# carlanton/cilium

Measured on AMD Instinct MI355X. Metric: Mpps classified (whole node) + % HBM roofline, 1/2/4/8 MI355X, higher is better.
Workload: dtype u32

## Files before the change

cilium_amd/csrc/gf_kernels.hip:

```cpp
#include "gf_internal.h"
#include "gf_device.h"
#include <rocprim/device/device_radix_sort.hpp>
#include <rocprim/device/device_scan.hpp>
#include <rocprim/device/device_run_length_encode.hpp>
#include <rocprim/device/device_select.hpp>
#include <rocprim/iterator/discard_iterator.hpp>
#include <rocprim/iterator/counting_iterator.hpp>
#include <errno.h>
#include <stdlib.h>
#include <stdio.h>
#include <functional>
#include <unordered_set>
#include <chrono>
#include <algorithm>
#include <array>
#include <atomic>
#include <string.h>

using namespace gf;
using namespace gfd;

#define BLOCK 256
#ifndef GF_DIAG
#define GF_DIAG 0
// ... 1668 lines not shown
    }
    if (stats && !(GF_DIAG & 2)) {
#if GF_ING_BINS_WAVE
        st.bins_wave(true, o.reason, o.action);
#else
        st.add(o.reason); st.add(256 + o.action);
#endif
        ln.sc.add(r.len, ab, o.ct_ret & 3u, st);
    }
}

__device__ __forceinline__ gf_rec ld_rec(const gf_rec *rec, uint32_t i) {
    if constexpr (GF_REC_NT) {
        const uint4 a = gload_nt16(rec + i), b = gload_nt16(reinterpret_cast<const uint8_t *>(rec + i) + 16);
        gf_rec r;
        __builtin_memcpy(&r, &a, 16);
        __builtin_memcpy(reinterpret_cast<uint8_t *>(&r) + 16, &b, 16);
        return r;
    } else {
        return rec[i];
    }
}
__device__ __forceinline__ void flush_added(const IngCtx &X, uint32_t fam_bit, int added, uint32_t *ct_count,
                                            uint32_t *lds_added) {
    if (X.strict & fam_bit) return;
    if (added) atomicAdd(lds_added, (uint32_t)added);
    __syncthreads();
    if (threadIdx.x == 0 && *lds_added && ct_count) atomicAdd(ct_count, *lds_added);
}

#ifndef GF_NCLS
#define GF_NCLS 1u
#endif
#define GF_NL (2u * GF_NCLS)
#define GF_LCAP 1024u
#define GF_SCHED_HIST(p) (p)
#define GF_SCHED_BASE(p) ((p) + GF_NL * (GF_LCAP + 1))
#define GF_SCHED_CURSOR(p) ((p) + 2 * GF_NL * (GF_LCAP + 1))
#define GF_SCHED_NRUNS(p) ((p) + 3 * GF_NL * (GF_LCAP + 1))
#define GF_SCHED_QUEUE(p) (GF_SCHED_NRUNS(p) + 1)
#define GF_SCHED_NFAM(p) (GF_SCHED_QUEUE(p) + GF_NL)
#define GF_SCHED_LCNT(p) (GF_SCHED_NFAM(p) + 2)
#define GF_SCHED_LSTART(p) (GF_SCHED_LCNT(p) + GF_NL)
#define GF_SCHED_WORDS (3 * GF_NL * (GF_LCAP + 1) + 1 + GF_NL + 2 + 2 * GF_NL)
#define GF_SCHED_HBYTES (GF_NL * (GF_LCAP + 1) * 4)
__device__ __forceinline__ uint32_t sched_list(uint32_t key, const gf_rec *rec, const uint32_t *perm, uint32_t b) {
    const uint32_t f = key >> (GF_KEY_BITS - 1);
    const uint32_t x = rec ? (uint32_t)rec[perm[b]].ep % GF_NCLS : 0u;
    return f * GF_NCLS + x;
}

template <int FAM, int GRAB = 1, bool PCT = false, bool RL = false>
__global__ __launch_bounds__(BLOCK, FAM == 6 ? GF_ING_MINW6 : GF_ING_MINW) void k_ing_groups(IngCtx X, uint32_t *sched, const uint2 *order,
                                                      const uint32_t *perm,
                                                      const gf_rec *rec, gf_ingress_out *out, uint32_t *ct_count,
                                                      unsigned long long *stats) {
    constexpr int F = FAM == 6 ? 1 : 0;
    const uint32_t *nfam = GF_SCHED_NFAM(sched);
    if (nfam[F] == 0) return;
    __shared__ uint32_t sl[272];
    __shared__ uint32_t sadd;
    Stats st{sl};
    if (threadIdx.x == 0) sadd = 0;
    if (stats) st.init(); else __syncthreads();
    const uint32_t lane = threadIdx.x & 63u;
    const uint32_t *lcnt = GF_SCHED_LCNT(sched), *lstart = GF_SCHED_LSTART(sched);
    __shared__ Lane<FAM> lanes[BLOCK];
    Lane<FAM> &ln = lanes[threadIdx.x];
    ln.init();
    uint32_t *const rlog = RL && X.rlog && !(X.rlog_off && *X.rlog_off) ? X.rlog : nullptr;
    const uint32_t x0 = blockIdx.x % GF_NCLS;
    for (uint32_t xi = 0; xi < GF_NCLS; xi++) {
    const uint32_t L = F * GF_NCLS + (x0 + xi) % GF_NCLS;
    uint32_t *queue = GF_SCHED_QUEUE(sched) + L;
    const uint32_t nb = lcnt[L];
    const uint2 *lorder = order + lstart[L];
    uint32_t grab = 1, gbase = 0, left = 0;
    for (;;) {
        uint32_t t;
        bool first = false;
        if constexpr (GRAB == 1) {
            uint32_t base = 0;
            if (lane == 0) base = atomicAdd(queue, 64u);
            base = __shfl(base, 0);
            if (base >= nb) break;
            t = base + lane;
        } else {
            if (!left) {
                uint32_t b0 = 0;
                if (lane == 0) b0 = atomicAdd(queue, 64u * grab);
                gbase = (uint32_t)__builtin_amdgcn_readfirstlane((int)b0);
                left = grab;
            }
            if (gbase >= nb) break;
            t = gbase + lane;
            first = left == grab;
            gbase += 64u; left--;
        }
        if (t >= nb) continue;
        const uint2 oc = lorder[t];
        if (GRAB > 1 && first && (uint32_t)__builtin_amdgcn_readfirstlane((int)oc.y) == 1u) grab = GRAB;
        const uint32_t b = oc.x, c = oc.y;
        uint32_t i = perm[b];
        uint32_t inx = c > 1 ? perm[b + 1] : 0u;
        gf_rec r = ld_rec(rec, i);
        lane_rel_drop<FAM, PCT>(X, ln);
// ... 135 lines not shown
        act = !(r.cls & 8) && (all || (r.ep && (gload<uint32_t>(&X.cfgs[r.ep - 1].flags) & GF_LXC_F_NO_CONNTRACK)));
        if (act) {
            len = r.len; ab = 8;
            o = handle_policy_noct(X, r, i, ab);
            if (X.pout && X.pout_wo) {
                uint8_t *q = X.pout + 24 * (size_t)i;
                const uint32_t ff = ((uint32_t)(r.cls >> 4) & 7u) << 5;
                *reinterpret_cast<uint32_t *>(q) = GF_STAGE_POLICY | ((uint32_t)o.action << 8) | ((uint32_t)o.reason << 16) |
                                                   ((uint32_t)o.ct_ret << 24);
                *reinterpret_cast<uint32_t *>(q + 4) = (ff | o.flags) | ((uint32_t)o.proxy_port << 16);
                *reinterpret_cast<uint16_t *>(q + 8) = o.ifindex_lo;
            } else if (X.pout) {
                uint8_t *q = X.pout + 24 * (size_t)i;
                uint2 a = *reinterpret_cast<const uint2 *>(q);
                uint2 b = *reinterpret_cast<const uint2 *>(q + 8);
                a.x = (a.x & 0xffu) | ((uint32_t)o.action << 8) | ((uint32_t)o.reason << 16) | ((uint32_t)o.ct_ret << 24);
                a.y = ((a.y & 0xffu) | o.flags) | (a.y & 0xff00u) | ((uint32_t)o.proxy_port << 16);
                b.x = (b.x & 0xffff0000u) | o.ifindex_lo;
                *reinterpret_cast<uint2 *>(q) = a;
                *reinterpret_cast<uint2 *>(q + 8) = b;
            } else {
                out[i] = o;
            }
        }
    }
    if (stats) {
        st.pkt_wave(act, o.reason, o.action, len, ab);
        const uint32_t c = (uint32_t)__popcll(__ballot(act));
        if ((threadIdx.x & 63u) == 0) st.add_n(264, c);
        st.flush(stats);
    }
}

#define GF_LCAP 1024u
#define GF_SCHED_ITEMS 4096
__global__ __launch_bounds__(BLOCK) void k_bucket_hist(uint32_t n, const uint32_t *off, const uint32_t *skeys,
                                                       const gf_rec *rec, const uint32_t *perm, uint32_t *sched) {
    extern __shared__ uint32_t h[];
    for (uint32_t k = threadIdx.x; k < GF_NL * (GF_LCAP + 1); k += blockDim.x) h[k] = 0;
    __syncthreads();
    uint32_t nq = *GF_SCHED_NRUNS(sched);
    uint32_t b0 = blockIdx.x * GF_SCHED_ITEMS;
    for (uint32_t q = b0 + threadIdx.x; q < b0 + GF_SCHED_ITEMS && q < nq; q += blockDim.x) {
        const uint32_t key = skeys[off[q]];
        uint32_t c = (q + 1 < nq ? off[q + 1] : n) - off[q];
        if (c && key != GF_KEY_SKIP)
            atomicAdd(&h[sched_list(key, rec, perm, off[q]) * (GF_LCAP + 1) + (c < GF_LCAP ? c : GF_LCAP)], 1u);
    }
    __syncthreads();
    uint32_t *hist = GF_SCHED_HIST(sched);
    for (uint32_t k = threadIdx.x; k < GF_NL * (GF_LCAP + 1); k += blockDim.x)
        if (h[k]) atomicAdd(&hist[k], h[k]);
}

__global__ __launch_bounds__(GF_LCAP) void k_bucket_base(uint32_t *sched) {
    __shared__ uint32_t s[GF_LCAP];
    __shared__ uint32_t tot;
    const uint32_t k = threadIdx.x, c = GF_LCAP - k;
    const uint32_t *hist = GF_SCHED_HIST(sched);
    uint32_t *base = GF_SCHED_BASE(sched), *cursor = GF_SCHED_CURSOR(sched);
    if (k == 0) { tot = 0; GF_SCHED_NFAM(sched)[0] = GF_SCHED_NFAM(sched)[1] = 0; }
    __syncthreads();
    for (uint32_t l = 0; l < GF_NL; l++) {
        const uint32_t *hf = hist + l * (GF_LCAP + 1);
        s[k] = hf[c];
        __syncthreads();
        for (uint32_t d = 1; d < GF_LCAP; d <<= 1) {
            uint32_t v = k >= d ? s[k - d] : 0u;
            __syncthreads();
            s[k] += v;
            __syncthreads();
        }
        const uint32_t add = tot;
        base[l * (GF_LCAP + 1) + c] = add + s[k] - hf[c];
        cursor[l * (GF_LCAP + 1) + c] = 0;
        if (k == 0) { base[l * (GF_LCAP + 1)] = add; cursor[l * (GF_LCAP + 1)] = 0; }
        __syncthreads();
        if (k == GF_LCAP - 1) {
            GF_SCHED_LCNT(sched)[l] = s[k];
            GF_SCHED_LSTART(sched)[l] = add;
            GF_SCHED_NFAM(sched)[l / GF_NCLS] += s[k];
            GF_SCHED_QUEUE(sched)[l] = 0;
            tot = add + s[k];
        }
        __syncthreads();
    }
}

__global__ __launch_bounds__(BLOCK) void k_bucket_order(uint32_t n, const uint32_t *off, const uint32_t *skeys,
                                                        const gf_rec *rec, const uint32_t *perm, uint32_t *sched,
                                                        uint2 *order, uint32_t skip1) {
    extern __shared__ uint32_t h[];
    for (uint32_t k = threadIdx.x; k < GF_NL * (GF_LCAP + 1); k += blockDim.x) h[k] = 0;
    __syncthreads();
    uint32_t nq = *GF_SCHED_NRUNS(sched);
    const uint32_t *base = GF_SCHED_BASE(sched);
    uint32_t *cursor = GF_SCHED_CURSOR(sched);
    uint32_t b0 = blockIdx.x * GF_SCHED_ITEMS;
    for (uint32_t q = b0 + threadIdx.x; q < b0 + GF_SCHED_ITEMS && q < nq; q += blockDim.x) {
        const uint32_t key = skeys[off[q]];
        uint32_t c = (q + 1 < nq ? off[q + 1] : n) - off[q];
        if (c && key != GF_KEY_SKIP && !(skip1 && c == 1))
            atomicAdd(&h[sched_list(key, rec, perm, off[q]) * (GF_LCAP + 1) + (c < GF_LCAP ? c : GF_LCAP)], 1u);
    }
    __syncthreads();
    for (uint32_t k = threadIdx.x; k < GF_NL * (GF_LCAP + 1); k += blockDim.x)
        if (h[k]) h[k] = base[k] + atomicAdd(&cursor[k], h[k]);
    __syncthreads();
    for (uint32_t q = b0 + threadIdx.x; q < b0 + GF_SCHED_ITEMS && q < nq; q += blockDim.x) {
        const uint32_t key = skeys[off[q]];
        uint32_t c = (q + 1 < nq ? off[q + 1] : n) - off[q];
        if (c && key != GF_KEY_SKIP && !(skip1 && c == 1))
            order[atomicAdd(&h[sched_list(key, rec, perm, off[q]) * (GF_LCAP + 1) + (c < GF_LCAP ? c : GF_LCAP)], 1u)] =
                make_uint2(off[q], c);
    }
}
__global__ __launch_bounds__(BLOCK) void k_single_mark(uint32_t n, const uint32_t *off, const uint32_t *skeys,
                                                       const uint32_t *perm, const uint32_t *sched, uint32_t *sw) {
    const uint32_t nq = *GF_SCHED_NRUNS(sched);
    for (uint32_t q = blockIdx.x * BLOCK + threadIdx.x; q < nq; q += gridDim.x * BLOCK) {
        const uint32_t b = off[q], key = skeys[b];
        if ((q + 1 < nq ? off[q + 1] : n) - b != 1u || key == GF_KEY_SKIP) continue;
        sw[perm[b]] = ((b + 1u) << 1) | (key >> (GF_KEY_BITS - 1));
    }
}
__device__ __forceinline__ uint32_t single_fam(uint32_t w) { return w ? 1u + (w & 1u) : 0u; }
__global__ __launch_bounds__(BLOCK) void k_single_count(uint32_t n, const uint32_t *sw, uint32_t *t0, uint32_t *t1) {
    __shared__ uint32_t wc[2][BLOCK / 64];
    const uint32_t b0 = blockIdx.x * GF_RUN_ITEMS, lane = threadIdx.x & 63u;
    uint32_t c0 = 0, c1 = 0;
    for (uint32_t k = 0; k < GF_RUN_ITEMS / BLOCK; k++) {
        const uint32_t j = b0 + k * BLOCK + threadIdx.x;
        const uint32_t f = j < n ? single_fam(sw[j]) : 0u;
        c0 += (uint32_t)__popcll(__ballot(f == 1u));
        c1 += (uint32_t)__popcll(__ballot(f == 2u));
    }
    if (lane == 0) { wc[0][threadIdx.x >> 6] = c0; wc[1][threadIdx.x >> 6] = c1; }
    __syncthreads();
    if (threadIdx.x == 0) {
        uint32_t a = 0, z = 0;
        for (uint32_t w = 0; w < BLOCK / 64; w++) { a += wc[0][w]; z += wc[1][w]; }
        t0[blockIdx.x] = a; t1[blockIdx.x] = z;
    }
}
__global__ __launch_bounds__(BLOCK) void k_single_write(uint32_t n, const uint32_t *sw, const uint32_t *t0,
                                                        const uint32_t *t1, const uint32_t *sched, uint2 *order) {
    __shared__ uint32_t wc[2][BLOCK / 64];
    const uint32_t b0 = blockIdx.x * GF_RUN_ITEMS, lane = threadIdx.x & 63u, wv = threadIdx.x >> 6;
    const uint32_t *base = GF_SCHED_BASE(sched);
    uint32_t p0 = base[0 * (GF_LCAP + 1) + 1] + t0[blockIdx.x], p1 = base[1 * (GF_LCAP + 1) + 1] + t1[blockIdx.x];
    for (uint32_t k = 0; k < GF_RUN_ITEMS / BLOCK; k++) {
        const uint32_t j = b0 + k * BLOCK + threadIdx.x;
        const uint32_t w = j < n ? sw[j] : 0u, f = single_fam(w);
        const uint64_t m0 = __ballot(f == 1u), m1 = __ballot(f == 2u);
        if (lane == 0) { wc[0][wv] = (uint32_t)__popcll(m0); wc[1][wv] = (uint32_t)__popcll(m1); }
        __syncthreads();
// ... 2540 lines not shown
            ifx = E.encap_ifindex;
            return TC_REDIRECT;
        }
    }
    const int r4 = eg_ipv6_l3(w, nullptr, nm);
    if (r4 != TC_OK) return r4;
    {
        const uint32_t old = w.r32(14) & __builtin_bswap32(0x0FF00000u);
        w.w32(14, __builtin_bswap32(0x60000000u) | __builtin_bswap32(gload<uint32_t>(&c->seclabel)) | old);
    }
    o.eg_flags |= GF_EG_F_TO_STACK;
    return TC_OK;
}

template <int FAM, bool PCT = false>
__global__ __launch_bounds__(BLOCK, GF_EG_MINW) void k_eg_groups(EgDev E, uint32_t *sched, const uint2 *order, const uint32_t *perm,
                                                     const EgRec *erec, gf_egress_out *out, gf_rec *rec2, uint32_t *key2,
                                                     uint32_t *ct_count, unsigned long long *stats) {
    if (E.hz && *E.hz) return;
    if (GF_EG_LEAN && !GF_SCHED_NFAM(sched)[FAM == 6 ? 1 : 0]) return;
    __shared__ uint32_t sl[272];
    __shared__ uint32_t sadd;
    extern __shared__ uint4 lds[];
    __shared__ uint32_t lsum[3 * BLOCK];
    Stats st{sl};
    uint32_t *ls = lsum + 3 * threadIdx.x;
    ls[0] = ls[1] = ls[2] = 0;
    auto fold = [&]() { st.add_n(268, ls[0]); st.add_n(269, ls[1]); st.add_n(270, ls[2]); ls[0] = ls[1] = ls[2] = 0; };
    if (threadIdx.x == 0) sadd = 0;
    if (stats) st.init(); else __syncthreads();
    const uint32_t K = eg_stage_bytes(E.stride);
    uint8_t *row = reinterpret_cast<uint8_t *>(lds) + (FAM == 6 ? 0 : threadIdx.x * eg_row_bytes(E.stride));
    constexpr int F = FAM == 6 ? 1 : 0;
    const uint32_t nb = GF_SCHED_LCNT(sched)[F * GF_NCLS], lane = threadIdx.x & 63u;
    uint32_t *queue = GF_SCHED_QUEUE(sched) + F * GF_NCLS;
    order += GF_SCHED_LSTART(sched)[F * GF_NCLS];
    const bool seq = *E.seq != 0;
    const bool rlog = FAM == 4 && E.conn && !seq && !*E.cflag;
    int added = 0;
    uint32_t grab = 1, base = 0, left = 0;
    for (;;) {
        if (!left) {
            uint32_t b0 = 0;
            if (lane == 0) b0 = atomicAdd(queue, 64u * grab);
            base = (uint32_t)__builtin_amdgcn_readfirstlane((int)b0);
            left = grab;
        }
        if (base >= nb) break;
        const uint32_t tq = base + lane;
        const bool first = left == grab;
        base += 64u; left--;
        if (tq >= nb) continue;
        const uint2 oc = order[tq];
        if (first && (uint32_t)__builtin_amdgcn_readfirstlane((int)oc.y) == 1u) grab = GF_GRAB_EG;
        for (uint32_t k = 0; k < oc.y; k++) {
            const uint32_t i = perm[oc.x + k];
            const EgRec r = erec[i];
            gf_rec rr;
            if (r.st) continue;
            gf_egress_out o{};
            o.stage = GF_STAGE_FROM_LXC;
            o.slave = r.slave; o.rev_nat = r.rev_nat; o.eg_flags = r.eflags;
            uint32_t ifx = 0, lxc = 0, ab = 24 + 34 + 32;
            uint8_t *g = E.snap + (size_t)i * E.stride;
            constexpr bool v6 = FAM == 6;
            int ret;
            PktHdr h2;
            if constexpr (v6) {
                Row w{g, E.stride < r.len ? E.stride : r.len};
// ... 179 lines not shown
    ProfEntry e{};
    bool on;
    hipStream_t s;
    ProfScope(const char *n, hipStream_t s_) : on(prof().on), s(s_) {
        if (!on) return;
        e.name = n;
        (void)hipEventCreateWithFlags(&e.a, hipEventDisableSystemFence);
        (void)hipEventCreateWithFlags(&e.b, hipEventDisableSystemFence);
        (void)hipEventRecord(e.a, s);
    }
    ~ProfScope() {
        if (!on) return;
        (void)hipEventRecord(e.b, s);
        std::lock_guard<std::mutex> g(prof().mu);
        prof().pending.push_back(e);
    }
};
void prof_drain() {
    std::lock_guard<std::mutex> g(prof().mu);
    for (auto &e : prof().pending) {
        float ms = 0;
        if (hipEventSynchronize(e.b) == hipSuccess && hipEventElapsedTime(&ms, e.a, e.b) == hipSuccess) {
            auto &a = prof().acc[e.name];
            a.first++;
            a.second += ms;
        }
        (void)hipEventDestroy(e.a);
        (void)hipEventDestroy(e.b);
    }
    prof().pending.clear();
}

struct Workspace {
    DevBuf rec, keys, skeys, perm, tcnt, off, tmp, sched, order;
    DevBuf sb, st0, st1;
};
struct HostMarks {
    using clk = std::chrono::steady_clock;
    bool on;
    clk::time_point t0, last;
    char buf[768];
    int len = 0;
    HostMarks *prev;
    static HostMarks *&cur() { static thread_local HostMarks *c = nullptr; return c; }
    HostMarks() : on(getenv("GF_HOST_PROF") != nullptr), prev(cur()) {
        buf[0] = 0;
        if (on) { t0 = last = clk::now(); cur() = this; }
    }
    static double us(clk::duration d) { return std::chrono::duration<double, std::micro>(d).count(); }
    void mark(const char *what) {
        if (!on) return;
        const auto t = clk::now();
        if (len < (int)sizeof buf - 40) len += snprintf(buf + len, sizeof buf - len, " %s %.0f", what, us(t - last));
        last = t;
    }
    ~HostMarks() {
        if (!on) return;
        cur() = prev;
        fprintf(stderr, "[gf] host us:%s | total %.0f\n", buf, us(clk::now() - t0));
    }
};
void host_mark(const char *what) { if (HostMarks *m = HostMarks::cur()) m->mark(what); }
}
namespace gf {
struct CallCtx {
    std::mutex mu;
    hipEvent_t ev = nullptr;
// ... 418 lines not shown
}

static int emit_drop_events(EvSrc E, hipStream_t s) {
    gf_event_ring R = event_ring();
    if (!R.records || !R.count || !R.capacity || E.n == 0) return 0;
    struct EvWs { DevBuf blk, boff, tmp; };
    static const char tag = 0;
    EvWs &ew = cur_ctx().get<EvWs>(&tag);
    DevBuf &blk = ew.blk, &boff = ew.boff, &tmp = ew.tmp;
    const uint32_t nb = (E.n + BLOCK - 1) / BLOCK;
    auto grow = [](DevBuf &d, size_t want) -> int { return d.bytes >= want ? 0 : d.ensure(want); };
    int r;
    if ((r = grow(blk, (size_t)nb * 4)) || (r = grow(boff, (size_t)nb * 4))) return r;
    size_t tb = 0;
    (void)rocprim::exclusive_scan(nullptr, tb, (uint32_t *)blk.p, (uint32_t *)boff.p, 0u, nb, rocprim::plus<uint32_t>(), s);
    if ((r = grow(tmp, tb + 256))) return r;
    ProfScope ps("k_drop_events", s);
    hipLaunchKernelGGL(k_ev_count, dim3(nb), dim3(BLOCK), 0, s, E, (uint32_t *)blk.p);
    tb = tmp.bytes;
    if (hip_ok(rocprim::exclusive_scan(tmp.p, tb, (uint32_t *)blk.p, (uint32_t *)boff.p, 0u, nb,
                                       rocprim::plus<uint32_t>(), s), "event scan"))
        return -EIO;
    hipLaunchKernelGGL(k_ev_write, dim3(nb), dim3(BLOCK), 0, s, E, (const uint32_t *)boff.p, R);
    hipLaunchKernelGGL(k_ev_commit, dim3(1), dim3(1), 0, s, (const uint32_t *)boff.p, (const uint32_t *)blk.p, nb, R);
    return hip_ok(hipGetLastError(), "k_drop_events");
}

static int ws_grow(uint32_t n) {
    Workspace &w = ws();
    auto grow = [](DevBuf &b, size_t want) -> int { return b.bytes >= want ? 0 : b.ensure(want); };
    int r;
    if ((r = grow(w.rec, (size_t)n * sizeof(gf_rec))) || (r = grow(w.keys, (size_t)n * 4)) ||
        (r = grow(w.skeys, (size_t)n * 4)) || (r = grow(w.perm, (size_t)n * 4 + 16)) ||
        (r = grow(w.off, (size_t)n * 4)) || (r = grow(w.order, (size_t)n * 8)) ||
        (r = grow(w.sched, GF_SCHED_WORDS * 4)))
        return r;
    return 0;
}

#ifndef GF_SORT_RADIX
#define GF_SORT_RADIX 8
#endif
#ifndef GF_SORT_IPT
#define GF_SORT_IPT 16
#endif
#if GF_SORT_RADIX == 8 && GF_SORT_IPT == 16
using GfSortCfg = rocprim::default_config;
#else
using GfSortCfg = rocprim::radix_sort_config<
    rocprim::default_config, rocprim::default_config,
    rocprim::radix_sort_onesweep_config<rocprim::kernel_config<1024, GF_SORT_IPT>, rocprim::kernel_config<1024, GF_SORT_IPT>,
                                        GF_SORT_RADIX, rocprim::block_radix_rank_algorithm::match>>;
#endif
__device__ __forceinline__ bool run_start(const uint32_t *k, uint32_t j) { return j == 0 || k[j] != k[j - 1]; }
__global__ __launch_bounds__(BLOCK) void k_run_count(uint32_t n, const uint32_t *skeys, uint32_t *tcnt,
                                                     uint32_t *zero = nullptr) {
    __shared__ uint32_t wc[BLOCK / 64];
    const uint32_t b0 = blockIdx.x * GF_RUN_ITEMS, lane = threadIdx.x & 63u;
    uint32_t c = 0;
    for (uint32_t k = 0; k < GF_RUN_ITEMS / BLOCK; k++) {
        const uint32_t j = b0 + k * BLOCK + threadIdx.x;
        c += (uint32_t)__popcll(__ballot(j < n && run_start(skeys, j)));
        if (zero && j < n) zero[j] = 0u;
    }
    if (lane == 0) wc[threadIdx.x >> 6] = c;
    __syncthreads();
    if (threadIdx.x == 0) {
        uint32_t t = 0;
        for (uint32_t w = 0; w < BLOCK / 64; w++) t += wc[w];
        tcnt[blockIdx.x] = t;
    }
}
__global__ __launch_bounds__(1024) void k_run_scan(uint32_t nt, uint32_t *tcnt, uint32_t *nruns, uint32_t *zero = nullptr,
                                                   uint32_t nzero = 0) {
    __shared__ uint32_t part[1024];
    __shared__ uint32_t carry;
    for (uint32_t k = threadIdx.x; k < nzero; k += 1024) zero[k] = 0;
    if (threadIdx.x == 0) carry = 0;
    __syncthreads();
    for (uint32_t c0 = 0; c0 < nt; c0 += 1024) {
        const uint32_t t = c0 + threadIdx.x;
        const uint32_t v = t < nt ? tcnt[t] : 0u;
        part[threadIdx.x] = v;
        __syncthreads();
        for (uint32_t o = 1; o < 1024; o <<= 1) {
            const uint32_t x = threadIdx.x >= o ? part[threadIdx.x - o] : 0u;
            __syncthreads();
            part[threadIdx.x] += x;
            __syncthreads();
        }
        if (t < nt) tcnt[t] = carry + part[threadIdx.x] - v;
        __syncthreads();
        if (threadIdx.x == 1023) carry += part[1023];
        __syncthreads();
    }
    if (threadIdx.x == 0) *nruns = carry;
}
__global__ __launch_bounds__(BLOCK) void k_run_write(uint32_t n, const uint32_t *skeys, const uint32_t *toff,
                                                     uint32_t *off) {
    __shared__ uint32_t wc[BLOCK / 64];
    const uint32_t b0 = blockIdx.x * GF_RUN_ITEMS, lane = threadIdx.x & 63u, wv = threadIdx.x >> 6;
    uint32_t base = toff[blockIdx.x];
    for (uint32_t k = 0; k < GF_RUN_ITEMS / BLOCK; k++) {
        const uint32_t j = b0 + k * BLOCK + threadIdx.x;
        const bool f = j < n && run_start(skeys, j);
        const uint64_t m = __ballot(f);
        if (lane == 0) wc[wv] = (uint32_t)__popcll(m);
        __syncthreads();
        uint32_t before = 0, all = 0;
        for (uint32_t w = 0; w < BLOCK / 64; w++) { before += w < wv ? wc[w] : 0u; all += wc[w]; }
        if (f) off[base + before + (uint32_t)__popcll(m & ((1ull << lane) - 1ull))] = j;
        base += all;
        __syncthreads();
    }
}
static int schedule_groups(uint32_t n, hipStream_t s, const gf_rec *rec = nullptr, bool single = false) {
    Workspace &w = ws();
    auto grow = [](DevBuf &b, size_t want) -> int { return b.bytes >= want ? 0 : b.ensure(want); };
    int r;
    uint32_t *d_sched = (uint32_t *)w.sched.p, *d_nruns = GF_SCHED_NRUNS(d_sched);
    size_t sort_bytes = 0;
    (void)rocprim::radix_sort_pairs<GfSortCfg>(nullptr, sort_bytes, (uint32_t *)w.keys.p, (uint32_t *)w.skeys.p,
                                               rocprim::counting_iterator<uint32_t>(0u), (uint32_t *)w.perm.p, n, 0,
                                               GF_KEY_BITS, s);
    const uint32_t nt = (n + GF_RUN_ITEMS - 1) / GF_RUN_ITEMS;
    if ((r = grow(w.tmp, sort_bytes + 256)) || (r = grow(w.tcnt, (size_t)nt * 4 + 16))) return r;
    single = single && GF_SINGLE_ORDER && GF_NCLS == 1;
    if (single && ((r = grow(w.sb, (size_t)n * 4)) || (r = grow(w.st0, (size_t)nt * 4 + 16)) ||
                   (r = grow(w.st1, (size_t)nt * 4 + 16))))
        return r;
    size_t tb = w.tmp.bytes;
    {
        ProfScope ps("rocprim_radix_sort", s);
        if (hip_ok(rocprim::radix_sort_pairs<GfSortCfg>(w.tmp.p, tb, (uint32_t *)w.keys.p, (uint32_t *)w.skeys.p,
                                                        rocprim::counting_iterator<uint32_t>(0u), (uint32_t *)w.perm.p,
                                                        n, 0, GF_KEY_BITS, s), "radix_sort_pairs"))
            return -EIO;
    }
    {
        ProfScope ps("bucket_runs", s);
        if (nt) hipLaunchKernelGGL(k_run_count, dim3(nt), dim3(BLOCK), 0, s, n, (const uint32_t *)w.skeys.p,
                                   (uint32_t *)w.tcnt.p, single ? (uint32_t *)w.sb.p : nullptr);
        hipLaunchKernelGGL(k_run_scan, dim3(1), dim3(1024), 0, s, nt, (uint32_t *)w.tcnt.p, d_nruns,
                           GF_SCHED_HIST(d_sched), GF_SCHED_HBYTES / 4u);
        if (nt) hipLaunchKernelGGL(k_run_write, dim3(nt), dim3(BLOCK), 0, s, n, (const uint32_t *)w.skeys.p,
                                   (const uint32_t *)w.tcnt.p, (uint32_t *)w.off.p);
        if ((r = hip_ok(hipGetLastError(), "run starts"))) return r;
    }
    {
        ProfScope ps("k_bucket_sched", s);
        static const bool lds_ok = [] {
            return hipFuncSetAttribute((const void *)k_bucket_hist, hipFuncAttributeMaxDynamicSharedMemorySize,
                                       (int)GF_SCHED_HBYTES) == hipSuccess &&
                   hipFuncSetAttribute((const void *)k_bucket_order, hipFuncAttributeMaxDynamicSharedMemorySize,
                                       (int)GF_SCHED_HBYTES) == hipSuccess;
        }();
        if (!lds_ok) return hip_ok(hipErrorInvalidValue, "k_bucket_sched LDS");
        uint32_t g = (n + GF_SCHED_ITEMS - 1) / GF_SCHED_ITEMS;
        const gf_rec *lrec = GF_NCLS > 1 ? rec : nullptr;
        hipLaunchKernelGGL(k_bucket_hist, dim3(g), dim3(BLOCK), GF_SCHED_HBYTES, s, n, (const uint32_t *)w.off.p,
                           (const uint32_t *)w.skeys.p, lrec, (const uint32_t *)w.perm.p, d_sched);
        hipLaunchKernelGGL(k_bucket_base, dim3(1), dim3(GF_LCAP), 0, s, d_sched);
        hipLaunchKernelGGL(k_bucket_order, dim3(g), dim3(BLOCK), GF_SCHED_HBYTES, s, n, (const uint32_t *)w.off.p,
                           (const uint32_t *)w.skeys.p, lrec, (const uint32_t *)w.perm.p, d_sched, (uint2 *)w.order.p,
                           single ? 1u : 0u);
        if (single) {
            hipLaunchKernelGGL(k_single_mark, dim3(std::min<uint32_t>((n + BLOCK - 1) / BLOCK, 8192u)), dim3(BLOCK), 0, s, n,
                               (const uint32_t *)w.off.p, (const uint32_t *)w.skeys.p, (const uint32_t *)w.perm.p,
                               (const uint32_t *)d_sched, (uint32_t *)w.sb.p);
            hipLaunchKernelGGL(k_single_count, dim3(nt), dim3(BLOCK), 0, s, n, (const uint32_t *)w.sb.p,
                               (uint32_t *)w.st0.p, (uint32_t *)w.st1.p);
            hipLaunchKernelGGL(k_run_scan, dim3(1), dim3(1024), 0, s, nt, (uint32_t *)w.st0.p, (uint32_t *)w.st0.p + nt,
                               nullptr, 0u);
            hipLaunchKernelGGL(k_run_scan, dim3(1), dim3(1024), 0, s, nt, (uint32_t *)w.st1.p, (uint32_t *)w.st1.p + nt,
                               nullptr, 0u);
            hipLaunchKernelGGL(k_single_write, dim3(nt), dim3(BLOCK), 0, s, n, (const uint32_t *)w.sb.p,
                               (const uint32_t *)w.st0.p, (const uint32_t *)w.st1.p, (const uint32_t *)d_sched,
                               (uint2 *)w.order.p);
        }
    }
    return hip_ok(hipGetLastError(), "k_bucket_sched");
}

struct PxWs {
    DevBuf plog, plog_n, pkey, pkey2, pval, pperm, ptmp;
    bool live = false;
};
static PxWs &px_ws() { static const char tag = 0; return cur_ctx().get<PxWs>(&tag); }
static int px_log_begin(uint32_t n, hipStream_t s, IngCtx &X, bool keep = false) {
    auto px4 = proxy_map(4), px6 = proxy_map(6);
    X.plog = nullptr; X.plog_n = nullptr;
    PxWs &w = px_ws();
    if (!px4 && !px6 && !X.snap && !(keep && w.live)) { w.live = keep && w.live; return 0; }
    int r;
    auto grow = [](DevBuf &b, size_t want) -> int { return b.bytes >= want ? 0 : b.ensure(want); };
    if ((r = grow(w.plog, (size_t)n * 64)) || (r = grow(w.plog_n, 4))) return r;
    if ((!keep || !w.live) && hip_ok(hipMemsetAsync(w.plog_n.p, 0, 4, s), "plog_n")) return -EIO;
    w.live = true;
    for (auto &m : {px4, px6})
        if (m && (r = push_map(m, s))) return r;
    X.plog = (uint32_t *)w.plog.p; X.plog_n = (uint32_t *)w.plog_n.p;
    return 0;
}
static int px_log_apply(const IngCtx &X, hipStream_t s, uint8_t *wsnap, const uint32_t *len, uint32_t stride,
                        uint8_t *recs, bool wide, uint32_t n) {
    if (!X.plog) return 0;
    px_ws().live = false;
    auto px4 = proxy_map(4), px6 = proxy_map(6);
// ... 1783 lines not shown
```

Before: 4299.

## Fuse run detection into per-tile schedule histogram and order kernels

Drops the separate run-count, run-scan and run-write passes and the global run-offset array. Each tile now finds its own run starts in LDS and feeds them straight into the bucket histogram and order scatter, and single-run marking moves into the order kernel. It adds replicated histogram copies to cut atomic contention, keeps the bins zeroed across calls instead of re-zeroing them each time, and adds an optional key-window split of the lists (off by default). The cost is extra run-boundary work at tile edges and larger static LDS use per block.

```diff
diff --git a/cilium_amd/csrc/gf_kernels.hip b/cilium_amd/csrc/gf_kernels.hip
--- a/cilium_amd/csrc/gf_kernels.hip
+++ b/cilium_amd/csrc/gf_kernels.hip
@@ -1724,22 +1724,30 @@
 #ifndef GF_NCLS
 #define GF_NCLS 1u
 #endif
-#define GF_NL (2u * GF_NCLS)
-#define GF_LCAP 1024u
+#ifndef GF_KWIN
+#define GF_KWIN 1u
+#endif
+static_assert(GF_KWIN >= 1u && (GF_KWIN & (GF_KWIN - 1u)) == 0u && GF_KWIN < GF_KEY_FAM, "GF_KWIN: a power of two");
+#define GF_NL (2u * GF_KWIN * GF_NCLS)
+#define GF_LIST(f, win, x) (((f) * GF_KWIN + (win)) * GF_NCLS + (x))
+#define GF_LCAP (GF_NL <= 2u ? 1024u : 8192u / GF_NL - 1u)
+#define GF_SCHED_BINS (GF_NL * (GF_LCAP + 1))
+#define GF_SREP (GF_KWIN >= 16u ? 1u : 16u / GF_KWIN)
 #define GF_SCHED_HIST(p) (p)
-#define GF_SCHED_BASE(p) ((p) + GF_NL * (GF_LCAP + 1))
-#define GF_SCHED_CURSOR(p) ((p) + 2 * GF_NL * (GF_LCAP + 1))
-#define GF_SCHED_NRUNS(p) ((p) + 3 * GF_NL * (GF_LCAP + 1))
+#define GF_SCHED_BASE(p) ((p) + GF_SREP * GF_SCHED_BINS)
+#define GF_SCHED_CURSOR(p) ((p) + 2 * GF_SREP * GF_SCHED_BINS)
+#define GF_SCHED_NRUNS(p) ((p) + 3 * GF_SREP * GF_SCHED_BINS)
 #define GF_SCHED_QUEUE(p) (GF_SCHED_NRUNS(p) + 1)
 #define GF_SCHED_NFAM(p) (GF_SCHED_QUEUE(p) + GF_NL)
 #define GF_SCHED_LCNT(p) (GF_SCHED_NFAM(p) + 2)
 #define GF_SCHED_LSTART(p) (GF_SCHED_LCNT(p) + GF_NL)
-#define GF_SCHED_WORDS (3 * GF_NL * (GF_LCAP + 1) + 1 + GF_NL + 2 + 2 * GF_NL)
-#define GF_SCHED_HBYTES (GF_NL * (GF_LCAP + 1) * 4)
-__device__ __forceinline__ uint32_t sched_list(uint32_t key, const gf_rec *rec, const uint32_t *perm, uint32_t b) {
+#define GF_SCHED_WORDS (3 * GF_SREP * GF_SCHED_BINS + 1 + GF_NL + 2 + 2 * GF_NL)
+__device__ __forceinline__ uint32_t sched_list(uint32_t key, const gf_rec *rec, const uint32_t *perm, uint32_t b,
+                                               bool win) {
     const uint32_t f = key >> (GF_KEY_BITS - 1);
     const uint32_t x = rec ? (uint32_t)rec[perm[b]].ep % GF_NCLS : 0u;
-    return f * GF_NCLS + x;
+    const uint32_t kw = GF_KWIN > 1u && win ? (key & GF_KEY_HASH) / (GF_KEY_FAM / GF_KWIN) : 0u;
+    return GF_LIST(f, kw, x);
 }
 
 template <int FAM, int GRAB = 1, bool PCT = false, bool RL = false>
@@ -1762,8 +1770,8 @@
     ln.init();
     uint32_t *const rlog = RL && X.rlog && !(X.rlog_off && *X.rlog_off) ? X.rlog : nullptr;
     const uint32_t x0 = blockIdx.x % GF_NCLS;
-    for (uint32_t xi = 0; xi < GF_NCLS; xi++) {
-    const uint32_t L = F * GF_NCLS + (x0 + xi) % GF_NCLS;
+    for (uint32_t li = 0; li < GF_KWIN * GF_NCLS; li++) {
+    const uint32_t L = GF_LIST(F, li / GF_NCLS, (x0 + li) % GF_NCLS);
     uint32_t *queue = GF_SCHED_QUEUE(sched) + L;
     const uint32_t nb = lcnt[L];
     const uint2 *lorder = order + lstart[L];
@@ -1965,38 +1973,109 @@
     }
 }
 
-#define GF_LCAP 1024u
-#define GF_SCHED_ITEMS 4096
-__global__ __launch_bounds__(BLOCK) void k_bucket_hist(uint32_t n, const uint32_t *off, const uint32_t *skeys,
-                                                       const gf_rec *rec, const uint32_t *perm, uint32_t *sched) {
-    extern __shared__ uint32_t h[];
-    for (uint32_t k = threadIdx.x; k < GF_NL * (GF_LCAP + 1); k += blockDim.x) h[k] = 0;
+static_assert(GF_RUN_ITEMS % (4 * BLOCK) == 0, "a tile is whole rounds of four keys per thread");
+#define GF_RUN_ROUNDS (GF_RUN_ITEMS / (4 * BLOCK))
+__device__ __forceinline__ uint32_t tile_runs(uint32_t n, const uint32_t *skeys, uint32_t *st, uint32_t *wc,
+                                              uint32_t *zero = nullptr) {
+    const uint32_t b0 = blockIdx.x * GF_RUN_ITEMS, lane = threadIdx.x & 63u, wv = threadIdx.x >> 6;
+    const uint64_t below = (1ull << lane) - 1ull;
+    uint32_t fl[GF_RUN_ROUNDS], pre[GF_RUN_ROUNDS];
+#pragma unroll
+    for (uint32_t k = 0; k < GF_RUN_ROUNDS; k++) {
+        const uint32_t j = b0 + (k * BLOCK + threadIdx.x) * 4u;
+        uint32_t v[4] = {0u, 0u, 0u, 0u}, f = 0;
+        if (j + 3u < n) {
+            const uint4 q = *reinterpret_cast<const uint4 *>(skeys + j);
+            v[0] = q.x; v[1] = q.y; v[2] = q.z; v[3] = q.w;
+            if (zero) *reinterpret_cast<uint4 *>(zero + j) = make_uint4(0u, 0u, 0u, 0u);
+        } else {
+            for (uint32_t e = 0; e < 4u; e++)
+                if (j + e < n) { v[e] = skeys[j + e]; if (zero) zero[j + e] = 0u; }
+        }
+        if (j < n) {
+            f = j == 0u || v[0] != skeys[j - 1u] ? 1u : 0u;
+            for (uint32_t e = 1; e < 4u; e++) f |= j + e < n && v[e] != v[e - 1u] ? 1u << e : 0u;
+        }
+        uint32_t p = 0, t = 0;
+#pragma unroll
+        for (uint32_t e = 0; e < 4u; e++) {
+            const uint64_t m = __ballot((f >> e) & 1u);
+            p += (uint32_t)__popcll(m & below); t += (uint32_t)__popcll(m);
+        }
+        fl[k] = f; pre[k] = p;
+        if (lane == 0) wc[k * (BLOCK / 64) + wv] = t;
+    }
     __syncthreads();
-    uint32_t nq = *GF_SCHED_NRUNS(sched);
-    uint32_t b0 = blockIdx.x * GF_SCHED_ITEMS;
-    for (uint32_t q = b0 + threadIdx.x; q < b0 + GF_SCHED_ITEMS && q < nq; q += blockDim.x) {
-        const uint32_t key = skeys[off[q]];
-        uint32_t c = (q + 1 < nq ? off[q + 1] : n) - off[q];
-        if (c && key != GF_KEY_SKIP)
-            atomicAdd(&h[sched_list(key, rec, perm, off[q]) * (GF_LCAP + 1) + (c < GF_LCAP ? c : GF_LCAP)], 1u);
-    }
+    uint32_t ns = 0, at[GF_RUN_ROUNDS];
+#pragma unroll
+    for (uint32_t k = 0; k < GF_RUN_ROUNDS; k++)
+        for (uint32_t w = 0; w < BLOCK / 64; w++) {
+            if (w == wv) at[k] = ns;
+            ns += wc[k * (BLOCK / 64) + w];
+        }
+#pragma unroll
+    for (uint32_t k = 0; k < GF_RUN_ROUNDS; k++) {
+        const uint32_t j = b0 + (k * BLOCK + threadIdx.x) * 4u;
+        uint32_t o = at[k] + pre[k];
+        for (uint32_t e = 0; e < 4u; e++)
+            if ((fl[k] >> e) & 1u) st[o++] = j + e;
+    }
+    if (threadIdx.x == 0) st[ns] = n;
     __syncthreads();
-    uint32_t *hist = GF_SCHED_HIST(sched);
-    for (uint32_t k = threadIdx.x; k < GF_NL * (GF_LCAP + 1); k += blockDim.x)
+    const uint32_t e0 = b0 + GF_RUN_ITEMS;
+    if (ns && e0 < n) {
+        const uint32_t j = e0 + threadIdx.x;
+        const bool f = j < n && skeys[j] != skeys[j - 1u];
+        if (__syncthreads_or(f)) {
+            if (f) atomicMin(&st[ns], j);
+        } else if (threadIdx.x == 0) {
+            const uint32_t key = skeys[e0 - 1u];
+            uint32_t lo = e0 + BLOCK < n ? e0 + BLOCK : n, hi = n;
+            while (lo < hi) {
+                const uint32_t mid = lo + (hi - lo) / 2u;
+                if (skeys[mid] == key) lo = mid + 1u; else hi = mid;
+            }
+            st[ns] = lo;
+        }
+        __syncthreads();
+    }
+    return ns;
+}
+__device__ __forceinline__ uint32_t sched_bin(uint32_t l, uint32_t c) { return l * (GF_LCAP + 1) + (c < GF_LCAP ? c : GF_LCAP); }
+
+__global__ __launch_bounds__(BLOCK) void k_sched_count(uint32_t n, const uint32_t *skeys, const gf_rec *rec,
+                                                       const uint32_t *perm, uint32_t *sched, bool win, uint32_t *zero) {
+    __shared__ uint32_t st[GF_RUN_ITEMS + 1], wc[GF_RUN_ROUNDS * (BLOCK / 64)], h[GF_SCHED_BINS];
+    for (uint32_t k = threadIdx.x; k < GF_SCHED_BINS; k += BLOCK) h[k] = 0;
+    const uint32_t ns = tile_runs(n, skeys, st, wc, zero);
+    for (uint32_t q = threadIdx.x; q < ns; q += BLOCK) {
+        const uint32_t b = st[q], c = st[q + 1] - b, key = skeys[b];
+        if (key != GF_KEY_SKIP) atomicAdd(&h[sched_bin(sched_list(key, rec, perm, b, win), c)], 1u);
+    }
+    __syncthreads();
+    uint32_t *hist = GF_SCHED_HIST(sched) + (blockIdx.x % GF_SREP) * GF_SCHED_BINS;
+    for (uint32_t k = threadIdx.x; k < GF_SCHED_BINS; k += BLOCK)
         if (h[k]) atomicAdd(&hist[k], h[k]);
 }
 
-__global__ __launch_bounds__(GF_LCAP) void k_bucket_base(uint32_t *sched) {
+__global__ __launch_bounds__(GF_LCAP) void k_sched_base(uint32_t *sched) {
     __shared__ uint32_t s[GF_LCAP];
     __shared__ uint32_t tot;
     const uint32_t k = threadIdx.x, c = GF_LCAP - k;
-    const uint32_t *hist = GF_SCHED_HIST(sched);
+    uint32_t *hist = GF_SCHED_HIST(sched);
     uint32_t *base = GF_SCHED_BASE(sched), *cursor = GF_SCHED_CURSOR(sched);
     if (k == 0) { tot = 0; GF_SCHED_NFAM(sched)[0] = GF_SCHED_NFAM(sched)[1] = 0; }
     __syncthreads();
     for (uint32_t l = 0; l < GF_NL; l++) {
-        const uint32_t *hf = hist + l * (GF_LCAP + 1);
-        s[k] = hf[c];
+        const uint32_t bin = l * (GF_LCAP + 1) + c;
+        uint32_t hr[GF_SREP], sum = 0;
+#pragma unroll
+        for (uint32_t r = 0; r < GF_SREP; r++) {
+            hr[r] = hist[r * GF_SCHED_BINS + bin];
+            hist[r * GF_SCHED_BINS + bin] = 0;
+            sum += hr[r];
+        }
+        s[k] = sum;
         __syncthreads();
         for (uint32_t d = 1; d < GF_LCAP; d <<= 1) {
             uint32_t v = k >= d ? s[k - d] : 0u;
@@ -2005,56 +2084,53 @@
             __syncthreads();
         }
         const uint32_t add = tot;
-        base[l * (GF_LCAP + 1) + c] = add + s[k] - hf[c];
-        cursor[l * (GF_LCAP + 1) + c] = 0;
-        if (k == 0) { base[l * (GF_LCAP + 1)] = add; cursor[l * (GF_LCAP + 1)] = 0; }
+        uint32_t at = add + s[k] - sum;
+#pragma unroll
+        for (uint32_t r = 0; r < GF_SREP; r++) {
+            base[r * GF_SCHED_BINS + bin] = at;
+            cursor[r * GF_SCHED_BINS + bin] = 0;
+            at += hr[r];
+        }
+        if (k == 0)
+            for (uint32_t r = 0; r < GF_SREP; r++) {
+                base[r * GF_SCHED_BINS + l * (GF_LCAP + 1)] = add;
+                cursor[r * GF_SCHED_BINS + l * (GF_LCAP + 1)] = 0;
+            }
         __syncthreads();
         if (k == GF_LCAP - 1) {
             GF_SCHED_LCNT(sched)[l] = s[k];
             GF_SCHED_LSTART(sched)[l] = add;
-            GF_SCHED_NFAM(sched)[l / GF_NCLS] += s[k];
+            GF_SCHED_NFAM(sched)[l / (GF_KWIN * GF_NCLS)] += s[k];
             GF_SCHED_QUEUE(sched)[l] = 0;
             tot = add + s[k];
+            if (l == GF_NL - 1) *GF_SCHED_NRUNS(sched) = tot;
         }
         __syncthreads();
     }
 }
 
-__global__ __launch_bounds__(BLOCK) void k_bucket_order(uint32_t n, const uint32_t *off, const uint32_t *skeys,
-                                                        const gf_rec *rec, const uint32_t *perm, uint32_t *sched,
-                                                        uint2 *order, uint32_t skip1) {
-    extern __shared__ uint32_t h[];
-    for (uint32_t k = threadIdx.x; k < GF_NL * (GF_LCAP + 1); k += blockDim.x) h[k] = 0;
+__global__ __launch_bounds__(BLOCK) void k_sched_order(uint32_t n, const uint32_t *skeys, const gf_rec *rec,
+                                                       const uint32_t *perm, uint32_t *sched, bool win, uint2 *order,
+                                                       uint32_t *sw) {
+    __shared__ uint32_t st[GF_RUN_ITEMS + 1], wc[GF_RUN_ROUNDS * (BLOCK / 64)], h[GF_SCHED_BINS];
+    for (uint32_t k = threadIdx.x; k < GF_SCHED_BINS; k += BLOCK) h[k] = 0;
+    const uint32_t ns = tile_runs(n, skeys, st, wc);
+    for (uint32_t q = threadIdx.x; q < ns; q += BLOCK) {
+        const uint32_t b = st[q], c = st[q + 1] - b, key = skeys[b];
+        if (key == GF_KEY_SKIP) continue;
+        if (sw && c == 1u) sw[perm[b]] = ((b + 1u) << 1) | (key >> (GF_KEY_BITS - 1));
+        else atomicAdd(&h[sched_bin(sched_list(key, rec, perm, b, win), c)], 1u);
+    }
     __syncthreads();
-    uint32_t nq = *GF_SCHED_NRUNS(sched);
-    const uint32_t *base = GF_SCHED_BASE(sched);
-    uint32_t *cursor = GF_SCHED_CURSOR(sched);
-    uint32_t b0 = blockIdx.x * GF_SCHED_ITEMS;
-    for (uint32_t q = b0 + threadIdx.x; q < b0 + GF_SCHED_ITEMS && q < nq; q += blockDim.x) {
-        const uint32_t key = skeys[off[q]];
-        uint32_t c = (q + 1 < nq ? off[q + 1] : n) - off[q];
-        if (c && key != GF_KEY_SKIP && !(skip1 && c == 1))
-            atomicAdd(&h[sched_list(key, rec, perm, off[q]) * (GF_LCAP + 1) + (c < GF_LCAP ? c : GF_LCAP)], 1u);
-    }
-    __syncthreads();
-    for (uint32_t k = threadIdx.x; k < GF_NL * (GF_LCAP + 1); k += blockDim.x)
+    const uint32_t *base = GF_SCHED_BASE(sched) + (blockIdx.x % GF_SREP) * GF_SCHED_BINS;
+    uint32_t *cursor = GF_SCHED_CURSOR(sched) + (blockIdx.x % GF_SREP) * GF_SCHED_BINS;
+    for (uint32_t k = threadIdx.x; k < GF_SCHED_BINS; k += BLOCK)
         if (h[k]) h[k] = base[k] + atomicAdd(&cursor[k], h[k]);
     __syncthreads();
-    for (uint32_t q = b0 + threadIdx.x; q < b0 + GF_SCHED_ITEMS && q < nq; q += blockDim.x) {
-        const uint32_t key = skeys[off[q]];
-        uint32_t c = (q + 1 < nq ? off[q + 1] : n) - off[q];
-        if (c && key != GF_KEY_SKIP && !(skip1 && c == 1))
-            order[atomicAdd(&h[sched_list(key, rec, perm, off[q]) * (GF_LCAP + 1) + (c < GF_LCAP ? c : GF_LCAP)], 1u)] =
-                make_uint2(off[q], c);
-    }
-}
-__global__ __launch_bounds__(BLOCK) void k_single_mark(uint32_t n, const uint32_t *off, const uint32_t *skeys,
-                                                       const uint32_t *perm, const uint32_t *sched, uint32_t *sw) {
-    const uint32_t nq = *GF_SCHED_NRUNS(sched);
-    for (uint32_t q = blockIdx.x * BLOCK + threadIdx.x; q < nq; q += gridDim.x * BLOCK) {
-        const uint32_t b = off[q], key = skeys[b];
-        if ((q + 1 < nq ? off[q + 1] : n) - b != 1u || key == GF_KEY_SKIP) continue;
-        sw[perm[b]] = ((b + 1u) << 1) | (key >> (GF_KEY_BITS - 1));
+    for (uint32_t q = threadIdx.x; q < ns; q += BLOCK) {
+        const uint32_t b = st[q], c = st[q + 1] - b, key = skeys[b];
+        if (key != GF_KEY_SKIP && !(sw && c == 1u))
+            order[atomicAdd(&h[sched_bin(sched_list(key, rec, perm, b, win), c)], 1u)] = make_uint2(b, c);
     }
 }
 __device__ __forceinline__ uint32_t single_fam(uint32_t w) { return w ? 1u + (w & 1u) : 0u; }
@@ -4661,9 +4737,9 @@
     const uint32_t K = eg_stage_bytes(E.stride);
     uint8_t *row = reinterpret_cast<uint8_t *>(lds) + (FAM == 6 ? 0 : threadIdx.x * eg_row_bytes(E.stride));
     constexpr int F = FAM == 6 ? 1 : 0;
-    const uint32_t nb = GF_SCHED_LCNT(sched)[F * GF_NCLS], lane = threadIdx.x & 63u;
-    uint32_t *queue = GF_SCHED_QUEUE(sched) + F * GF_NCLS;
-    order += GF_SCHED_LSTART(sched)[F * GF_NCLS];
+    const uint32_t nb = GF_SCHED_LCNT(sched)[GF_LIST(F, 0, 0)], lane = threadIdx.x & 63u;
+    uint32_t *queue = GF_SCHED_QUEUE(sched) + GF_LIST(F, 0, 0);
+    order += GF_SCHED_LSTART(sched)[GF_LIST(F, 0, 0)];
     const bool seq = *E.seq != 0;
     const bool rlog = FAM == 4 && E.conn && !seq && !*E.cflag;
     int added = 0;
@@ -4909,7 +4985,8 @@
 }
 
 struct Workspace {
-    DevBuf rec, keys, skeys, perm, tcnt, off, tmp, sched, order;
+    DevBuf rec, keys, skeys, perm, tmp, sched, order;
+    bool sched_zeroed = false;
     DevBuf sb, st0, st1;
 };
 struct HostMarks {
@@ -5394,9 +5471,12 @@
     int r;
     if ((r = grow(w.rec, (size_t)n * sizeof(gf_rec))) || (r = grow(w.keys, (size_t)n * 4)) ||
         (r = grow(w.skeys, (size_t)n * 4)) || (r = grow(w.perm, (size_t)n * 4 + 16)) ||
-        (r = grow(w.off, (size_t)n * 4)) || (r = grow(w.order, (size_t)n * 8)) ||
-        (r = grow(w.sched, GF_SCHED_WORDS * 4)))
+        (r = grow(w.order, (size_t)n * 8)))
         return r;
+    if (w.sched.bytes < GF_SCHED_WORDS * 4) {
+        w.sched_zeroed = false;
+        if ((r = w.sched.ensure(GF_SCHED_WORDS * 4))) return r;
+    }
     return 0;
 }
 
@@ -5414,30 +5494,9 @@
     rocprim::radix_sort_onesweep_config<rocprim::kernel_config<1024, GF_SORT_IPT>, rocprim::kernel_config<1024, GF_SORT_IPT>,
                                         GF_SORT_RADIX, rocprim::block_radix_rank_algorithm::match>>;
 #endif
-__device__ __forceinline__ bool run_start(const uint32_t *k, uint32_t j) { return j == 0 || k[j] != k[j - 1]; }
-__global__ __launch_bounds__(BLOCK) void k_run_count(uint32_t n, const uint32_t *skeys, uint32_t *tcnt,
-                                                     uint32_t *zero = nullptr) {
-    __shared__ uint32_t wc[BLOCK / 64];
-    const uint32_t b0 = blockIdx.x * GF_RUN_ITEMS, lane = threadIdx.x & 63u;
-    uint32_t c = 0;
-    for (uint32_t k = 0; k < GF_RUN_ITEMS / BLOCK; k++) {
-        const uint32_t j = b0 + k * BLOCK + threadIdx.x;
-        c += (uint32_t)__popcll(__ballot(j < n && run_start(skeys, j)));
-        if (zero && j < n) zero[j] = 0u;
-    }
-    if (lane == 0) wc[threadIdx.x >> 6] = c;
-    __syncthreads();
-    if (threadIdx.x == 0) {
-        uint32_t t = 0;
-        for (uint32_t w = 0; w < BLOCK / 64; w++) t += wc[w];
-        tcnt[blockIdx.x] = t;
-    }
-}
-__global__ __launch_bounds__(1024) void k_run_scan(uint32_t nt, uint32_t *tcnt, uint32_t *nruns, uint32_t *zero = nullptr,
-                                                   uint32_t nzero = 0) {
+__global__ __launch_bounds__(1024) void k_run_scan(uint32_t nt, uint32_t *tcnt, uint32_t *nruns) {
     __shared__ uint32_t part[1024];
     __shared__ uint32_t carry;
-    for (uint32_t k = threadIdx.x; k < nzero; k += 1024) zero[k] = 0;
     if (threadIdx.x == 0) carry = 0;
     __syncthreads();
     for (uint32_t c0 = 0; c0 < nt; c0 += 1024) {
@@ -5458,36 +5517,18 @@
     }
     if (threadIdx.x == 0) *nruns = carry;
 }
-__global__ __launch_bounds__(BLOCK) void k_run_write(uint32_t n, const uint32_t *skeys, const uint32_t *toff,
-                                                     uint32_t *off) {
-    __shared__ uint32_t wc[BLOCK / 64];
-    const uint32_t b0 = blockIdx.x * GF_RUN_ITEMS, lane = threadIdx.x & 63u, wv = threadIdx.x >> 6;
-    uint32_t base = toff[blockIdx.x];
-    for (uint32_t k = 0; k < GF_RUN_ITEMS / BLOCK; k++) {
-        const uint32_t j = b0 + k * BLOCK + threadIdx.x;
-        const bool f = j < n && run_start(skeys, j);
-        const uint64_t m = __ballot(f);
-        if (lane == 0) wc[wv] = (uint32_t)__popcll(m);
-        __syncthreads();
-        uint32_t before = 0, all = 0;
-        for (uint32_t w = 0; w < BLOCK / 64; w++) { before += w < wv ? wc[w] : 0u; all += wc[w]; }
-        if (f) off[base + before + (uint32_t)__popcll(m & ((1ull << lane) - 1ull))] = j;
-        base += all;
-        __syncthreads();
-    }
-}
 static int schedule_groups(uint32_t n, hipStream_t s, const gf_rec *rec = nullptr, bool single = false) {
     Workspace &w = ws();
     auto grow = [](DevBuf &b, size_t want) -> int { return b.bytes >= want ? 0 : b.ensure(want); };
     int r;
-    uint32_t *d_sched = (uint32_t *)w.sched.p, *d_nruns = GF_SCHED_NRUNS(d_sched);
+    uint32_t *d_sched = (uint32_t *)w.sched.p;
     size_t sort_bytes = 0;
     (void)rocprim::radix_sort_pairs<GfSortCfg>(nullptr, sort_bytes, (uint32_t *)w.keys.p, (uint32_t *)w.skeys.p,
                                                rocprim::counting_iterator<uint32_t>(0u), (uint32_t *)w.perm.p, n, 0,
                                                GF_KEY_BITS, s);
     const uint32_t nt = (n + GF_RUN_ITEMS - 1) / GF_RUN_ITEMS;
-    if ((r = grow(w.tmp, sort_bytes + 256)) || (r = grow(w.tcnt, (size_t)nt * 4 + 16))) return r;
-    single = single && GF_SINGLE_ORDER && GF_NCLS == 1;
+    if ((r = grow(w.tmp, sort_bytes + 256))) return r;
+    single = single && GF_SINGLE_ORDER && GF_NL == 2 && nt;
     if (single && ((r = grow(w.sb, (size_t)n * 4)) || (r = grow(w.st0, (size_t)nt * 4 + 16)) ||
                    (r = grow(w.st1, (size_t)nt * 4 + 16))))
         return r;
@@ -5499,43 +5540,30 @@
                                                         n, 0, GF_KEY_BITS, s), "radix_sort_pairs"))
             return -EIO;
     }
+    const gf_rec *lrec = GF_NCLS > 1 ? rec : nullptr;
+    const bool win = rec != nullptr;
+    uint32_t *sw = single ? (uint32_t *)w.sb.p : nullptr;
     {
         ProfScope ps("bucket_runs", s);
-        if (nt) hipLaunchKernelGGL(k_run_count, dim3(nt), dim3(BLOCK), 0, s, n, (const uint32_t *)w.skeys.p,
-                                   (uint32_t *)w.tcnt.p, single ? (uint32_t *)w.sb.p : nullptr);
-        hipLaunchKernelGGL(k_run_scan, dim3(1), dim3(1024), 0, s, nt, (uint32_t *)w.tcnt.p, d_nruns,
-                           GF_SCHED_HIST(d_sched), GF_SCHED_HBYTES / 4u);
-        if (nt) hipLaunchKernelGGL(k_run_write, dim3(nt), dim3(BLOCK), 0, s, n, (const uint32_t *)w.skeys.p,
-                                   (const uint32_t *)w.tcnt.p, (uint32_t *)w.off.p);
-        if ((r = hip_ok(hipGetLastError(), "run starts"))) return r;
+        if (!w.sched_zeroed &&
+            (r = hip_ok(hipMemsetAsync(GF_SCHED_HIST(d_sched), 0, GF_SREP * GF_SCHED_BINS * 4, s), "schedule bins")))
+            return r;
+        w.sched_zeroed = false;
+        if (nt) hipLaunchKernelGGL(k_sched_count, dim3(nt), dim3(BLOCK), 0, s, n, (const uint32_t *)w.skeys.p, lrec,
+                                   (const uint32_t *)w.perm.p, d_sched, win, sw);
+        hipLaunchKernelGGL(k_sched_base, dim3(1), dim3(GF_LCAP), 0, s, d_sched);
+        if ((r = hip_ok(hipGetLastError(), "bucket_runs"))) return r;
+        w.sched_zeroed = true;
     }
     {
         ProfScope ps("k_bucket_sched", s);
-        static const bool lds_ok = [] {
-            return hipFuncSetAttribute((const void *)k_bucket_hist, hipFuncAttributeMaxDynamicSharedMemorySize,
-                                       (int)GF_SCHED_HBYTES) == hipSuccess &&
-                   hipFuncSetAttribute((const void *)k_bucket_order, hipFuncAttributeMaxDynamicSharedMemorySize,
-                                       (int)GF_SCHED_HBYTES) == hipSuccess;
-        }();
-        if (!lds_ok) return hip_ok(hipErrorInvalidValue, "k_bucket_sched LDS");
-        uint32_t g = (n + GF_SCHED_ITEMS - 1) / GF_SCHED_ITEMS;
-        const gf_rec *lrec = GF_NCLS > 1 ? rec : nullptr;
-        hipLaunchKernelGGL(k_bucket_hist, dim3(g), dim3(BLOCK), GF_SCHED_HBYTES, s, n, (const uint32_t *)w.off.p,
-                           (const uint32_t *)w.skeys.p, lrec, (const uint32_t *)w.perm.p, d_sched);
-        hipLaunchKernelGGL(k_bucket_base, dim3(1), dim3(GF_LCAP), 0, s, d_sched);
-        hipLaunchKernelGGL(k_bucket_order, dim3(g), dim3(BLOCK), GF_SCHED_HBYTES, s, n, (const uint32_t *)w.off.p,
-                           (const uint32_t *)w.skeys.p, lrec, (const uint32_t *)w.perm.p, d_sched, (uint2 *)w.order.p,
-                           single ? 1u : 0u);
+        if (nt) hipLaunchKernelGGL(k_sched_order, dim3(nt), dim3(BLOCK), 0, s, n, (const uint32_t *)w.skeys.p, lrec,
+                                   (const uint32_t *)w.perm.p, d_sched, win, (uint2 *)w.order.p, sw);
         if (single) {
-            hipLaunchKernelGGL(k_single_mark, dim3(std::min<uint32_t>((n + BLOCK - 1) / BLOCK, 8192u)), dim3(BLOCK), 0, s, n,
-                               (const uint32_t *)w.off.p, (const uint32_t *)w.skeys.p, (const uint32_t *)w.perm.p,
-                               (const uint32_t *)d_sched, (uint32_t *)w.sb.p);
             hipLaunchKernelGGL(k_single_count, dim3(nt), dim3(BLOCK), 0, s, n, (const uint32_t *)w.sb.p,
                                (uint32_t *)w.st0.p, (uint32_t *)w.st1.p);
-            hipLaunchKernelGGL(k_run_scan, dim3(1), dim3(1024), 0, s, nt, (uint32_t *)w.st0.p, (uint32_t *)w.st0.p + nt,
-                               nullptr, 0u);
-            hipLaunchKernelGGL(k_run_scan, dim3(1), dim3(1024), 0, s, nt, (uint32_t *)w.st1.p, (uint32_t *)w.st1.p + nt,
-                               nullptr, 0u);
+            hipLaunchKernelGGL(k_run_scan, dim3(1), dim3(1024), 0, s, nt, (uint32_t *)w.st0.p, (uint32_t *)w.st0.p + nt);
+            hipLaunchKernelGGL(k_run_scan, dim3(1), dim3(1024), 0, s, nt, (uint32_t *)w.st1.p, (uint32_t *)w.st1.p + nt);
             hipLaunchKernelGGL(k_single_write, dim3(nt), dim3(BLOCK), 0, s, n, (const uint32_t *)w.sb.p,
                                (const uint32_t *)w.st0.p, (const uint32_t *)w.st1.p, (const uint32_t *)d_sched,
                                (uint2 *)w.order.p);
```

Measured after the change: 4335, median of 6. About the same (+0.9%).
